# LingmaFuture/PRCV2025REID

Measured on AMD Instinct MI355X. Metric: multimodal instances/sec (PxK, 5-modality) at 1/2/4/8 GPU; eval queries/sec, higher is better.
Workload: dtype bf16; 1 GPU; P=16,K=4 per GPU, vis/nir/sk/cp 224x224 + text (T<=77), CLIP ViT-B/16 + text tower random-init, MER-LoRA r=8, masks all-on, 400 ids, SDM+CE, fwd+bwd+grad sanitise/clip+AdamW (reference default trainable set); P=16, K=4, global_batch=64, lora_rank=8, accum_steps=1, parallelism=dp1

## Files before the change

prcv2025reid_amd/csrc/attention.hip:

```cpp
#include "common.h"
#include <stdlib.h>

namespace {

typedef __attribute__((ext_vector_type(4))) short s4;
typedef __attribute__((address_space(3))) s4* lds_s4_ptr;

constexpr float LOG2E = 1.4426950408889634f;

__device__ __forceinline__ int swz(int row, int c) { return c ^ ((row >> 1) & 7); }

typedef const __attribute__((address_space(1))) void* gptr_t;
typedef __attribute__((address_space(3))) void* lptr_t;

template <int NT>
__device__ __forceinline__ void stage_head(const bf16_t* __restrict__ base, int ld, int S, char* lds, int wave, int lane,
                                           int row_limit = 1 << 30) {
#pragma unroll
    for (int i = 0; i < 4; ++i) {
        const int rblk = (i * NT + wave) * 8;
        if (rblk >= row_limit) continue;
        const int row = rblk + (lane >> 3);
        const int c = swz(row, lane & 7);
        const int grow = row < S ? row : S - 1;
        __builtin_amdgcn_global_load_lds((gptr_t)(base + (size_t)grow * ld + c * 8), (lptr_t)(lds + rblk * 128), 16, 0, 0);
    }
}

__device__ __forceinline__ bf16x8 row_frag(const char* img, int row0, int kchunk, int lane) {
    const int row = row0 + (lane & 31);
    return *(const bf16x8*)(img + row * 128 + (swz(row, kchunk + (lane >> 5)) << 4));
}

__device__ __forceinline__ bf16x8 col_frag(const char* img, int krow0, int col0, int lane) {
    const int h = lane >> 5, half16 = (lane >> 4) & 1, i = lane & 15;
    const int q = i >> 2, pp = i & 3;
    const int col = col0 + 16 * half16 + 4 * pp;
    const int r_lo = krow0 + 4 * h + q, r_hi = r_lo + 8;
    const char* a_lo = img + r_lo * 128 + (swz(r_lo, col >> 3) << 4) + (col & 7) * 2;
    const char* a_hi = img + r_hi * 128 + (swz(r_hi, col >> 3) << 4) + (col & 7) * 2;
    const s4 lo = __builtin_amdgcn_ds_read_tr16_b64_v4i16((lds_s4_ptr)a_lo);
    const s4 hi = __builtin_amdgcn_ds_read_tr16_b64_v4i16((lds_s4_ptr)a_hi);
    return bf16x8{lo[0], lo[1], lo[2], lo[3], hi[0], hi[1], hi[2], hi[3]};
}

__device__ __forceinline__ bf16x8 gfrag(const bf16_t* __restrict__ base, int ld, int row, int kchunk, int lane) {
    return *(const bf16x8*)(base + (size_t)row * ld + (kchunk + (lane >> 5)) * 8);
}

struct FragOff {
    int row[4];
    int col_lo[2];
    int col_hi[2];
};
__device__ __forceinline__ FragOff make_frag_off(int lane) {
    FragOff f;
    const int r = lane & 31, h = lane >> 5;
#pragma unroll
    for (int ks = 0; ks < 4; ++ks) f.row[ks] = r * 128 + (swz(r, 2 * ks + h) << 4);
    const int half16 = (lane >> 4) & 1, i = lane & 15, q = i >> 2, pp = i & 3;
    const int r_lo = 4 * h + q, r_hi = r_lo + 8;
#pragma unroll
    for (int dt = 0; dt < 2; ++dt) {
        const int col = dt * 32 + 16 * half16 + 4 * pp;
        f.col_lo[dt] = r_lo * 128 + (swz(r_lo, col >> 3) << 4) + (col & 7) * 2;
        f.col_hi[dt] = r_hi * 128 + (swz(r_hi, col >> 3) << 4) + (col & 7) * 2;
    }
    return f;
}
__device__ __forceinline__ bf16x8 row_frag_o(const char* img, int tile_row0, int ks, const FragOff& f) {
    return *(const bf16x8*)(img + tile_row0 * 128 + f.row[ks]);
}
__device__ __forceinline__ bf16x8 col_frag_o(const char* img, int krow0, int dt, const FragOff& f) {
    const s4 lo = __builtin_amdgcn_ds_read_tr16_b64_v4i16((lds_s4_ptr)(img + krow0 * 128 + f.col_lo[dt]));
    const s4 hi = __builtin_amdgcn_ds_read_tr16_b64_v4i16((lds_s4_ptr)(img + krow0 * 128 + f.col_hi[dt]));
    return bf16x8{lo[0], lo[1], lo[2], lo[3], hi[0], hi[1], hi[2], hi[3]};
}
__device__ __forceinline__ float fast_exp2(float x) { return __builtin_amdgcn_exp2f(x); }

__device__ __forceinline__ bf16x8 pack8(const f32x16& a, int s) {
    bf16x8 r;
#pragma unroll
    for (int j = 0; j < 8; ++j) r[j] = (short)f32_to_bf16(a[8 * s + j]);
    return r;
}

__device__ __forceinline__ int acc_row(int reg, int lane) { return (reg & 3) + 8 * (reg >> 2) + 4 * (lane >> 5); }

struct AttnParams {
    const bf16_t* qkv; int ld; const uint8_t* key_mask;
    bf16_t* out; int ldo; float* lse;
    const bf16_t* dout; bf16_t* dqkv; int lddqkv; float* delta;
    int n_seq, S, heads, causal;
    int q_tiles;
};

__device__ __forceinline__ void store_tile_row16(bf16_t* row, bool ok, const f32x16& t, float scale, int lane) {
#pragma unroll
    for (int j = 0; j < 2; ++j) {
        const int a = 8 * j, b = 8 * j + 4;
        const auto r0 = __builtin_amdgcn_permlane32_swap(pack_bf16x2(t[a] * scale, t[a + 1] * scale),
                                                         pack_bf16x2(t[b] * scale, t[b + 1] * scale), false, false);
        const auto r1 = __builtin_amdgcn_permlane32_swap(pack_bf16x2(t[a + 2] * scale, t[a + 3] * scale),
                                                         pack_bf16x2(t[b + 2] * scale, t[b + 3] * scale), false, false);
        if (ok) *(uint4*)(row + 8 * (2 * j + (lane >> 5))) = uint4{r0[0], r1[0], r0[1], r1[1]};
    }
}


template <int NT, bool TWO_PASS>
__global__ __launch_bounds__(NT * 64, TWO_PASS ? 4 : 1) void attn_fwd_kernel(const AttnParams p) {
    REID_T16_ENTER();
    extern __shared__ __attribute__((aligned(16))) char smem[];
    char* Ks = smem;
    char* Vs = smem + NT * 32 * 128;
    const int tid = threadIdx.x, lane = tid & 63;
    const int wave = __builtin_amdgcn_readfirstlane(tid >> 6);
    const int seq = blockIdx.x / p.heads, head = blockIdx.x % p.heads;
    const int d = p.heads * 64;
    const bf16_t* qb = p.qkv + (size_t)seq * p.S * p.ld + head * 64;
    stage_head<NT>(qb + d, p.ld, p.S, Ks, wave, lane);
    const int q0 = wave * 32;
    const int qi = q0 + (lane & 31);
    const int qrow = qi < p.S ? qi : p.S - 1;
    bf16x8 qf[4];
#pragma unroll
    for (int ks = 0; ks < 4; ++ks) qf[ks] = gfrag(qb, p.ld, qrow, 2 * ks, lane);
    stage_head<NT>(qb + 2 * d, p.ld, p.S, Vs, wave, lane);
    __syncthreads();
    if (q0 >= p.S || (p.q_tiles > 0 && wave >= p.q_tiles)) return;

    const FragOff fo = make_frag_off(lane);
    const uint8_t* km = p.key_mask ? p.key_mask + (size_t)seq * p.S : nullptr;
    const int h4 = 4 * (lane >> 5);
    const bool general = km != nullptr || p.causal;
    auto score_tile = [&](int kt) -> f32x16 {
        f32x16 t;
#pragma unroll
        for (int e = 0; e < 16; ++e) t[e] = 0.f;
#pragma unroll
        for (int ks = 0; ks < 4; ++ks) t = mfma32(row_frag_o(Ks, kt * 32, ks, fo), qf[ks], t);
        if (general) {
#pragma unroll
            for (int e = 0; e < 16; ++e) {
                const int key = kt * 32 + (e & 3) + 8 * (e >> 2) + h4;
                bool ok = key < p.S;
                if (ok && km) ok = km[key] != 0;
                if (p.causal) ok = ok && key <= qi;
                t[e] = ok ? t[e] : -INFINITY;
            }
        } else if (kt == NT - 1) {
#pragma unroll
            for (int e = 0; e < 16; ++e) {
                const int key = kt * 32 + (e & 3) + 8 * (e >> 2) + h4;
                t[e] = key < p.S ? t[e] : -INFINITY;
            }
        }
        return t;
    };
    const float c = 0.125f * LOG2E;
    f32x16 ot[2];
#pragma unroll
    for (int dt = 0; dt < 2; ++dt)
#pragma unroll
        for (int e = 0; e < 16; ++e) ot[dt][e] = 0.f;
    float mx = -INFINITY, l = 0.f;
    if (TWO_PASS) {
#pragma unroll 1
        for (int kt = 0; kt < NT; ++kt) {
            const f32x16 t = score_tile(kt);
#pragma unroll
            for (int e = 0; e < 16; e += 2) mx = fmaxf(mx, fmaxf(t[e], t[e + 1]));
        }
        mx = fmaxf(mx, __shfl_xor(mx, 32, 64));
        if (mx == -INFINITY) mx = 0.f;
        const float nmc = -mx * c;
#pragma unroll 1
        for (int kt = 0; kt < NT; ++kt) {
            f32x16 t = score_tile(kt);
#pragma unroll
            for (int e = 0; e < 16; ++e) {
                const float pe = fast_exp2(fmaf(t[e], c, nmc));
                t[e] = pe;
                l += pe;
            }
#pragma unroll
            for (int s2 = 0; s2 < 2; ++s2) {
                const bf16x8 pf = pack8(t, s2);
#pragma unroll
                for (int dt = 0; dt < 2; ++dt) ot[dt] = mfma32(col_frag_o(Vs, kt * 32 + 16 * s2, dt, fo), pf, ot[dt]);
            }
        }
    } else {
        f32x16 st[NT];
#pragma unroll
        for (int kt = 0; kt < NT; ++kt) st[kt] = score_tile(kt);
#pragma unroll
        for (int kt = 0; kt < NT; ++kt)
#pragma unroll
            for (int e = 0; e < 16; e += 2) mx = fmaxf(mx, fmaxf(st[kt][e], st[kt][e + 1]));
        mx = fmaxf(mx, __shfl_xor(mx, 32, 64));
        if (mx == -INFINITY) mx = 0.f;
        const float nmc = -mx * c;
#pragma unroll
        for (int kt = 0; kt < NT; ++kt)
#pragma unroll
            for (int e = 0; e < 16; ++e) {
                const float pe = fast_exp2(fmaf(st[kt][e], c, nmc));
                st[kt][e] = pe;
                l += pe;
            }
#pragma unroll
        for (int kt = 0; kt < NT; ++kt)
#pragma unroll
            for (int s2 = 0; s2 < 2; ++s2) {
                const bf16x8 pf = pack8(st[kt], s2);
#pragma unroll
                for (int dt = 0; dt < 2; ++dt) ot[dt] = mfma32(col_frag_o(Vs, kt * 32 + 16 * s2, dt, fo), pf, ot[dt]);
            }
    }
    l += __shfl_xor(l, 32, 64);
    {
        const float inv = 1.0f / l;
        bf16_t* orow = p.out + ((size_t)seq * p.S + qrow) * p.ldo + head * 64;
#pragma unroll
        for (int dt = 0; dt < 2; ++dt) store_tile_row16(orow + dt * 32, qi < p.S, ot[dt], inv, lane);
        if (qi < p.S && p.lse && lane < 32) p.lse[((size_t)seq * p.heads + head) * p.S + qi] = mx * 0.125f + logf(l);
    }
}

template <int NT>
__global__ __launch_bounds__(NT * 64) void attn_bwd_dkv_kernel(const AttnParams p) {
    REID_T16_ENTER();
    extern __shared__ __attribute__((aligned(16))) char smem[];
    char* Qs = smem;
    char* Gs = smem + NT * 32 * 128;
    float* rowc = (float*)(smem + 2 * NT * 32 * 128);
    const int tid = threadIdx.x, lane = tid & 63;
    const int wave = __builtin_amdgcn_readfirstlane(tid >> 6);
    const int seq = blockIdx.x / p.heads, head = blockIdx.x % p.heads;
    const int d = p.heads * 64;
    const bf16_t* qb = p.qkv + (size_t)seq * p.S * p.ld + head * 64;
    const bf16_t* gb = p.dout + (size_t)seq * p.S * p.ldo + head * 64;
    const int q_rows = p.q_tiles > 0 ? p.q_tiles * 32 : NT * 32;
    stage_head<NT>(qb, p.ld, p.S, Qs, wave, lane, q_rows);
    stage_head<NT>(gb, p.ldo, p.S, Gs, wave, lane, q_rows);
    for (int t = tid; t < NT * 32; t += NT * 64) {
        const size_t o = ((size_t)seq * p.heads + head) * p.S + t;
        rowc[t] = t < p.S ? -p.lse[o] * LOG2E : -INFINITY;
        rowc[NT * 32 + t] = t < p.S ? -p.delta[o] * 0.125f : 0.f;
    }
    const int k0 = wave * 32;
    const int ki = k0 + (lane & 31);
    const int krow = ki < p.S ? ki : p.S - 1;
    bf16x8 kf[4], vf[4];
#pragma unroll
    for (int ks = 0; ks < 4; ++ks) {
        kf[ks] = gfrag(qb + d, p.ld, krow, 2 * ks, lane);
        vf[ks] = gfrag(qb + 2 * d, p.ld, krow, 2 * ks, lane);
    }
    __syncthreads();
    if (k0 >= p.S) return;
    const uint8_t* km = p.key_mask ? p.key_mask + (size_t)seq * p.S : nullptr;
    const bool key_ok = ki < p.S && (!km || km[ki] != 0);

    const FragOff fo = make_frag_off(lane);
    f32x16 dkt[2], dvt[2];
#pragma unroll
    for (int dt = 0; dt < 2; ++dt)
#pragma unroll
        for (int e = 0; e < 16; ++e) { dkt[dt][e] = 0.f; dvt[dt][e] = 0.f; }
    const float c = 0.125f * LOG2E;
    const int h4 = 4 * (lane >> 5);
    for (int qt = 0; qt < NT; ++qt) {
        if (qt * 32 >= p.S || (p.q_tiles > 0 && qt >= p.q_tiles)) break;
        f32x16 s, dp;
#pragma unroll
        for (int e = 0; e < 16; ++e) { s[e] = 0.f; dp[e] = 0.f; }
#pragma unroll
        for (int ks = 0; ks < 4; ++ks) {
            s = mfma32(row_frag_o(Qs, qt * 32, ks, fo), kf[ks], s);
            dp = mfma32(row_frag_o(Gs, qt * 32, ks, fo), vf[ks], dp);
        }
        f32x16 pm, ds;
#pragma unroll
        for (int g = 0; g < 4; ++g) {
            const f32x4 nl = *(const f32x4*)(rowc + qt * 32 + 8 * g + h4);
            const f32x4 nd = *(const f32x4*)(rowc + NT * 32 + qt * 32 + 8 * g + h4);
#pragma unroll
            for (int j = 0; j < 4; ++j) {
                const int e = 4 * g + j;
                float pe = fast_exp2(fmaf(s[e], c, nl[j]));
                if (p.causal && ki > qt * 32 + 8 * g + h4 + j) pe = 0.f;
                pm[e] = pe;
                ds[e] = pe * fmaf(dp[e], 0.125f, nd[j]);
            }
        }
#pragma unroll
        for (int s2 = 0; s2 < 2; ++s2) {
            const bf16x8 pf = pack8(pm, s2), df = pack8(ds, s2);
#pragma unroll
            for (int dt = 0; dt < 2; ++dt) {
                dvt[dt] = mfma32(col_frag_o(Gs, qt * 32 + 16 * s2, dt, fo), pf, dvt[dt]);
                dkt[dt] = mfma32(col_frag_o(Qs, qt * 32 + 16 * s2, dt, fo), df, dkt[dt]);
            }
        }
    }
    if (!key_ok) {
#pragma unroll
        for (int dt = 0; dt < 2; ++dt)
#pragma unroll
            for (int e = 0; e < 16; ++e) { dkt[dt][e] = 0.f; dvt[dt][e] = 0.f; }
    }
    {
        const bool ok = ki < p.S;
        bf16_t* drow = p.dqkv + ((size_t)seq * p.S + (ok ? ki : 0)) * p.lddqkv + head * 64;
#pragma unroll
        for (int dt = 0; dt < 2; ++dt) {
            store_tile_row16(drow + d + dt * 32, ok, dkt[dt], 1.0f, lane);
            store_tile_row16(drow + 2 * d + dt * 32, ok, dvt[dt], 1.0f, lane);
        }
    }
}

template <int NT>
__global__ __launch_bounds__(NT * 64) void attn_bwd_dq_kernel(const AttnParams p) {
    REID_T16_ENTER();
    extern __shared__ __attribute__((aligned(16))) char smem[];
    char* Ks = smem;
    char* Vs = smem + NT * 32 * 128;
    const int tid = threadIdx.x, lane = tid & 63;
    const int wave = __builtin_amdgcn_readfirstlane(tid >> 6);
    const int seq = blockIdx.x / p.heads, head = blockIdx.x % p.heads;
    const int d = p.heads * 64;
    const bf16_t* qb = p.qkv + (size_t)seq * p.S * p.ld + head * 64;
    const bf16_t* gb = p.dout + (size_t)seq * p.S * p.ldo + head * 64;
    stage_head<NT>(qb + d, p.ld, p.S, Ks, wave, lane);
    stage_head<NT>(qb + 2 * d, p.ld, p.S, Vs, wave, lane);
    const int q0 = wave * 32;
    const int qi = q0 + (lane & 31);
    const int qrow = qi < p.S ? qi : p.S - 1;
    bf16x8 qf[4], gf[4];
#pragma unroll
    for (int ks = 0; ks < 4; ++ks) {
        qf[ks] = gfrag(qb, p.ld, qrow, 2 * ks, lane);
        gf[ks] = gfrag(gb, p.ldo, qrow, 2 * ks, lane);
    }
    const size_t so = ((size_t)seq * p.heads + head) * p.S + qrow;
    const float nl = -p.lse[so] * LOG2E;
    float dsum = 0.f;
    {
        const bf16_t* ob = p.out + (size_t)seq * p.S * p.ldo + head * 64;
#pragma unroll
        for (int ks = 0; ks < 4; ++ks) {
            const bf16x8 of = gfrag(ob, p.ldo, qrow, 2 * ks, lane);
#pragma unroll
            for (int j = 0; j < 8; ++j) dsum = fmaf(bf16_to_f32((bf16_t)gf[ks][j]), bf16_to_f32((bf16_t)of[j]), dsum);
        }
    }
    dsum += __shfl_xor(dsum, 32, 64);
    if (qi < p.S && lane < 32) p.delta[so] = dsum;
    const float nd = -dsum * 0.125f;
    __syncthreads();
    if (q0 >= p.S) return;
    if (p.q_tiles > 0 && wave >= p.q_tiles) {
        if (qi < p.S) {
            bf16_t* drow = p.dqkv + ((size_t)seq * p.S + qi) * p.lddqkv + head * 64;
#pragma unroll
            for (int dt = 0; dt < 2; ++dt)
#pragma unroll
                for (int g = 0; g < 4; ++g) *(uint2*)(drow + dt * 32 + 8 * g + 4 * (lane >> 5)) = uint2{0u, 0u};
        }
        return;
    }
    const uint8_t* km = p.key_mask ? p.key_mask + (size_t)seq * p.S : nullptr;
    const FragOff fo = make_frag_off(lane);
    f32x16 dqt[2];
#pragma unroll
    for (int dt = 0; dt < 2; ++dt)
#pragma unroll
        for (int e = 0; e < 16; ++e) dqt[dt][e] = 0.f;
    const float c = 0.125f * LOG2E;
    const int h4 = 4 * (lane >> 5);
    const bool slow = km != nullptr || p.causal;
    for (int kt = 0; kt < NT; ++kt) {
        if (kt * 32 >= p.S) break;
        f32x16 s, dp;
#pragma unroll
        for (int e = 0; e < 16; ++e) { s[e] = 0.f; dp[e] = 0.f; }
#pragma unroll
        for (int ks = 0; ks < 4; ++ks) {
            s = mfma32(row_frag_o(Ks, kt * 32, ks, fo), qf[ks], s);
            dp = mfma32(row_frag_o(Vs, kt * 32, ks, fo), gf[ks], dp);
        }
        const bool edge = slow || (kt + 1) * 32 > p.S;
        f32x16 ds;
#pragma unroll
        for (int e = 0; e < 16; ++e) {
            float pe = fast_exp2(fmaf(s[e], c, nl));
            if (edge) {
                const int key = kt * 32 + (e & 3) + 8 * (e >> 2) + h4;
                bool ok = key < p.S;
                if (ok && km) ok = km[key] != 0;
                if (p.causal) ok = ok && key <= qi;
                pe = ok ? pe : 0.f;
            }
            ds[e] = pe * fmaf(dp[e], 0.125f, nd);
        }
#pragma unroll
        for (int s2 = 0; s2 < 2; ++s2) {
            const bf16x8 df = pack8(ds, s2);
#pragma unroll
            for (int dt = 0; dt < 2; ++dt) dqt[dt] = mfma32(col_frag_o(Ks, kt * 32 + 16 * s2, dt, fo), df, dqt[dt]);
        }
    }
    {
        const bool ok = qi < p.S;
        bf16_t* drow = p.dqkv + ((size_t)seq * p.S + (ok ? qi : 0)) * p.lddqkv + head * 64;
#pragma unroll
        for (int dt = 0; dt < 2; ++dt) store_tile_row16(drow + dt * 32, ok, dqt[dt], 1.0f, lane);
    }
}

#ifdef REID_ATTN_TRACE
__device__ unsigned long long* g_attn_bwd_trace = nullptr;
#define ATTN_BWD_STAMP(slot) do { if (g_attn_bwd_trace && threadIdx.x == 0) g_attn_bwd_trace[(size_t)blockIdx.x * 8 + (slot)] = __builtin_amdgcn_s_memrealtime(); } while (0)
#else
#define ATTN_BWD_STAMP(slot) do { } while (0)
#endif
template <int NT>
__global__ __launch_bounds__(NT * 64) void attn_bwd_fused_kernel(const AttnParams p) {
    REID_T16_ENTER();
    ATTN_BWD_STAMP(0);
    extern __shared__ __attribute__((aligned(16))) char smem[];
    constexpr int IMG = NT * 32 * 128;
    char* Qs = smem;
    char* Gs = smem + IMG;
    char* Ks = smem + 2 * IMG;
    char* Vs = smem + 3 * IMG;
    float* rowc = (float*)(smem + 4 * IMG);
    const int tid = threadIdx.x, lane = tid & 63;
    const int wave = __builtin_amdgcn_readfirstlane(tid >> 6);
    const int seq = blockIdx.x / p.heads, head = blockIdx.x % p.heads;
    const int d = p.heads * 64;
    const bf16_t* qb = p.qkv + (size_t)seq * p.S * p.ld + head * 64;
    const bf16_t* gb = p.dout + (size_t)seq * p.S * p.ldo + head * 64;
    const bf16_t* ob = p.out + (size_t)seq * p.S * p.ldo + head * 64;
    const int nq = p.q_tiles > 0 ? (p.q_tiles < NT ? p.q_tiles : NT) : NT;
    const int q_rows = nq * 32;
    stage_head<NT>(qb, p.ld, p.S, Qs, wave, lane, q_rows);
    stage_head<NT>(gb, p.ldo, p.S, Gs, wave, lane, q_rows);
    stage_head<NT>(qb + d, p.ld, p.S, Ks, wave, lane);
    stage_head<NT>(qb + 2 * d, p.ld, p.S, Vs, wave, lane);
    const int t0 = wave * 32;
    const int ti = t0 + (lane & 31);
    const int trow = ti < p.S ? ti : p.S - 1;
    const bool own_q = wave < nq && t0 < p.S;
    bf16x8 of[4];
#pragma unroll
    for (int ks = 0; ks < 4; ++ks) of[ks] = gfrag(ob, p.ldo, trow, 2 * ks, lane);
    const size_t so = ((size_t)seq * p.heads + head) * p.S + trow;
    const float lse_v = p.lse[so];
    const FragOff fo = make_frag_off(lane);
    __syncthreads();
    ATTN_BWD_STAMP(1);
    {
        float dsum = 0.f;
        if (own_q) {
#pragma unroll
            for (int ks = 0; ks < 4; ++ks) {
                const bf16x8 gfk = row_frag_o(Gs, t0, ks, fo);
#pragma unroll
                for (int j = 0; j < 8; ++j) dsum = fmaf(bf16_to_f32((bf16_t)gfk[j]), bf16_to_f32((bf16_t)of[ks][j]), dsum);
            }
        }
        dsum += __shfl_xor(dsum, 32, 64);
        if (lane < 32) {
            const bool live = own_q && ti < p.S;
            rowc[ti] = live ? -lse_v * LOG2E : -INFINITY;
            rowc[NT * 32 + ti] = live ? -dsum * 0.125f : 0.f;
            if (live && p.delta) p.delta[so] = dsum;
        }
    }
    __syncthreads();
    ATTN_BWD_STAMP(2);
    if (t0 >= p.S) return;
    const float c = 0.125f * LOG2E;
    const int h4 = 4 * (lane >> 5);
    const bool tile_ok = ti < p.S;

    {
        bf16x8 kf[4], vf[4];
#pragma unroll
        for (int ks = 0; ks < 4; ++ks) { kf[ks] = row_frag_o(Ks, t0, ks, fo); vf[ks] = row_frag_o(Vs, t0, ks, fo); }
        f32x16 dkt[2], dvt[2];
#pragma unroll
        for (int dt = 0; dt < 2; ++dt)
#pragma unroll
            for (int e = 0; e < 16; ++e) { dkt[dt][e] = 0.f; dvt[dt][e] = 0.f; }
        const int nqt = nq < (p.S + 31) / 32 ? nq : (p.S + 31) / 32;
        auto scores = [&](int qt, f32x16& s, f32x16& dp) {
#pragma unroll
            for (int e = 0; e < 16; ++e) { s[e] = 0.f; dp[e] = 0.f; }
#pragma unroll
            for (int ks = 0; ks < 4; ++ks) {
                s = mfma32(row_frag_o(Qs, qt * 32, ks, fo), kf[ks], s);
                dp = mfma32(row_frag_o(Gs, qt * 32, ks, fo), vf[ks], dp);
            }
        };
        f32x16 s, dp, s_n, dp_n;
        if (nqt > 0) scores(0, s, dp);
        for (int qt = 0; qt < nqt; ++qt) {
            if (qt + 1 < nqt) scores(qt + 1, s_n, dp_n);
#pragma unroll
            for (int s2 = 0; s2 < 2; ++s2) {
                bf16x8 pf, df;
#pragma unroll
                for (int g2 = 0; g2 < 2; ++g2) {
                    const int g = 2 * s2 + g2;
                    const f32x4 nl = *(const f32x4*)(rowc + qt * 32 + 8 * g + h4);
                    const f32x4 nd = *(const f32x4*)(rowc + NT * 32 + qt * 32 + 8 * g + h4);
#pragma unroll
                    for (int j = 0; j < 4; ++j) {
                        const int e = 4 * g + j;
                        const float pe = fast_exp2(fmaf(s[e], c, nl[j]));
                        pf[4 * g2 + j] = (short)f32_to_bf16(pe);
                        df[4 * g2 + j] = (short)f32_to_bf16(pe * fmaf(dp[e], 0.125f, nd[j]));
                    }
                }
#pragma unroll
                for (int dt = 0; dt < 2; ++dt) {
                    dvt[dt] = mfma32(col_frag_o(Gs, qt * 32 + 16 * s2, dt, fo), pf, dvt[dt]);
                    dkt[dt] = mfma32(col_frag_o(Qs, qt * 32 + 16 * s2, dt, fo), df, dkt[dt]);
                }
            }
            s = s_n; dp = dp_n;
        }
        ATTN_BWD_STAMP(3);
        bf16_t* drow = p.dqkv + ((size_t)seq * p.S + trow) * p.lddqkv + head * 64;
#pragma unroll
        for (int dt = 0; dt < 2; ++dt) {
            store_tile_row16(drow + d + dt * 32, tile_ok, dkt[dt], 1.0f, lane);
            store_tile_row16(drow + 2 * d + dt * 32, tile_ok, dvt[dt], 1.0f, lane);
        }
    }

    ATTN_BWD_STAMP(4);
    bf16_t* qrow_out = p.dqkv + ((size_t)seq * p.S + trow) * p.lddqkv + head * 64;
    if (!own_q) {
        if (tile_ok) {
#pragma unroll
            for (int dt = 0; dt < 2; ++dt)
#pragma unroll
                for (int g = 0; g < 4; ++g) *(uint2*)(qrow_out + dt * 32 + 8 * g + 4 * (lane >> 5)) = uint2{0u, 0u};
        }
        return;
    }
    {
        bf16x8 qf[4], gf[4];
#pragma unroll
        for (int ks = 0; ks < 4; ++ks) { qf[ks] = row_frag_o(Qs, t0, ks, fo); gf[ks] = row_frag_o(Gs, t0, ks, fo); }
        const float nl = rowc[ti], nd = rowc[NT * 32 + ti];
        f32x16 dqt[2];
#pragma unroll
        for (int dt = 0; dt < 2; ++dt)
#pragma unroll
            for (int e = 0; e < 16; ++e) dqt[dt][e] = 0.f;
        const int nkt = (p.S + 31) / 32;
        auto scores_t = [&](int kt, f32x16& s, f32x16& dp) {
#pragma unroll
            for (int e = 0; e < 16; ++e) { s[e] = 0.f; dp[e] = 0.f; }
#pragma unroll
            for (int ks = 0; ks < 4; ++ks) {
                s = mfma32(row_frag_o(Ks, kt * 32, ks, fo), qf[ks], s);
                dp = mfma32(row_frag_o(Vs, kt * 32, ks, fo), gf[ks], dp);
            }
        };
        f32x16 s, dp, s_n, dp_n;
        scores_t(0, s, dp);
        for (int kt = 0; kt < nkt; ++kt) {
            if (kt + 1 < nkt) scores_t(kt + 1, s_n, dp_n);
            const bool edge = (kt + 1) * 32 > p.S;
#pragma unroll
            for (int s2 = 0; s2 < 2; ++s2) {
                bf16x8 df;
#pragma unroll
                for (int j = 0; j < 8; ++j) {
                    const int e = 8 * s2 + j;
                    float pe = fast_exp2(fmaf(s[e], c, nl));
                    if (edge) {
                        const int key = kt * 32 + (e & 3) + 8 * (e >> 2) + h4;
                        pe = key < p.S ? pe : 0.f;
                    }
                    df[j] = (short)f32_to_bf16(pe * fmaf(dp[e], 0.125f, nd));
                }
#pragma unroll
                for (int dt = 0; dt < 2; ++dt) dqt[dt] = mfma32(col_frag_o(Ks, kt * 32 + 16 * s2, dt, fo), df, dqt[dt]);
            }
            s = s_n; dp = dp_n;
        }
        ATTN_BWD_STAMP(5);
#pragma unroll
        for (int dt = 0; dt < 2; ++dt) store_tile_row16(qrow_out + dt * 32, tile_ok, dqt[dt], 1.0f, lane);
        ATTN_BWD_STAMP(6);
    }
}

template <int NT>
int launch_fwd(const AttnParams& p, hipStream_t s) {
    constexpr int LDS = 2 * NT * 32 * 128;
    constexpr bool TP = NT >= 4;
    REID_MAX_LDS((attn_fwd_kernel<NT, TP>), LDS);
    hipLaunchKernelGGL((attn_fwd_kernel<NT, TP>), dim3(p.n_seq * p.heads), dim3(NT * 64), LDS, s, p);
    REID_CHECK_LAUNCH("reid_attn_fwd");
    return REID_OK;
}

template <int NT>
int launch_bwd(const AttnParams& p, hipStream_t s) {
    constexpr int LDS1 = 2 * NT * 32 * 128 + 2 * NT * 32 * 4;
    constexpr int LDS2 = 2 * NT * 32 * 128;
    REID_MAX_LDS((attn_bwd_dkv_kernel<NT>), LDS1);
    REID_MAX_LDS((attn_bwd_dq_kernel<NT>), LDS2);
    if (!p.key_mask && !p.causal && reid_knob(KNOB_ATTN_BWD) != 1) {
        constexpr int LDSF = 4 * NT * 32 * 128 + 2 * NT * 32 * 4;
        REID_MAX_LDS((attn_bwd_fused_kernel<NT>), LDSF);
        hipLaunchKernelGGL(attn_bwd_fused_kernel<NT>, dim3(p.n_seq * p.heads), dim3(NT * 64), LDSF, s, p);
        REID_CHECK_LAUNCH("reid_attn_bwd(fused)");
        return REID_OK;
    }
    hipLaunchKernelGGL(attn_bwd_dq_kernel<NT>, dim3(p.n_seq * p.heads), dim3(NT * 64), LDS2, s, p);
    REID_CHECK_LAUNCH("reid_attn_bwd(dq)");
    hipLaunchKernelGGL(attn_bwd_dkv_kernel<NT>, dim3(p.n_seq * p.heads), dim3(NT * 64), LDS1, s, p);
    REID_CHECK_LAUNCH("reid_attn_bwd(dkv)");
    return REID_OK;
}

int check_common(const char* name, const void* qkv, int ld, int n_seq, int S, int heads) {
    REID_CHECK_ARG(qkv != nullptr, "%s: null qkv", name);
    REID_CHECK_ARG(n_seq > 0 && heads > 0 && S > 0 && S <= 224, "%s: S=%d must be in 1..224 (n_seq=%d heads=%d)", name, S, n_seq, heads);
    REID_CHECK_ARG(ld >= 3 * heads * 64 && ld % 8 == 0, "%s: ld=%d must be >= 3*heads*64 and a multiple of 8", name, ld);
    return REID_OK;
}

}

#ifdef REID_ATTN_TRACE
extern "C" void reid_debug_attn_bwd_trace(void* buf) {
    unsigned long long* ptr = (unsigned long long*)buf;
    (void)hipMemcpyToSymbol(HIP_SYMBOL(g_attn_bwd_trace), &ptr, sizeof(ptr));
}
#endif

#define DISPATCH_NT(nt, fn, ...)                \
    switch (nt) {                               \
        case 1: return fn<1>(__VA_ARGS__);      \
        case 2: return fn<2>(__VA_ARGS__);      \
        case 3: return fn<3>(__VA_ARGS__);      \
        case 4: return fn<4>(__VA_ARGS__);      \
        case 5: return fn<5>(__VA_ARGS__);      \
        case 6: return fn<6>(__VA_ARGS__);      \
        default: return fn<7>(__VA_ARGS__);     \
    }

extern "C" int reid_attn_fwd(const void* qkv, int32_t ld, const uint8_t* key_mask, void* out, int32_t ldo, float* lse,
                             int32_t n_seq, int32_t S, int32_t heads, int32_t causal, int32_t q_tiles, void* stream) {
    int rc = check_common("reid_attn_fwd", qkv, ld, n_seq, S, heads);
    if (rc) return rc;
    REID_CHECK_ARG(out && ldo >= heads * 64 && ldo % 4 == 0, "reid_attn_fwd: out/ldo");
    AttnParams p{(const bf16_t*)qkv, ld, key_mask, (bf16_t*)out, ldo, lse, nullptr, nullptr, 0, nullptr, n_seq, S, heads, causal, q_tiles};
    DISPATCH_NT((S + 31) / 32, launch_fwd, p, (hipStream_t)stream)
}

extern "C" int reid_attn_bwd(const void* qkv, int32_t ld, const uint8_t* key_mask, const void* out, const void* dout,
                             int32_t ldo, const float* lse, void* dqkv, int32_t lddqkv, float* delta_ws, int32_t n_seq,
                             int32_t S, int32_t heads, int32_t causal, int32_t q_tiles, void* stream) {
    int rc = check_common("reid_attn_bwd", qkv, ld, n_seq, S, heads);
    if (rc) return rc;
    REID_CHECK_ARG(out && dout && lse && dqkv && delta_ws, "reid_attn_bwd: null pointer");
    REID_CHECK_ARG(ldo >= heads * 64 && ldo % 8 == 0 && lddqkv >= 3 * heads * 64 && lddqkv % 4 == 0, "reid_attn_bwd: ldo/lddqkv");
    AttnParams p{(const bf16_t*)qkv, ld, key_mask, (bf16_t*)out, ldo, (float*)lse, (const bf16_t*)dout, (bf16_t*)dqkv, lddqkv,
                 delta_ws, n_seq, S, heads, causal, q_tiles};
    DISPATCH_NT((S + 31) / 32, launch_bwd, p, (hipStream_t)stream)
}
```

Baseline: 2072 instances/s.

## Reuse dS from dK/dV pass for dQ via LDS transpose reads

The fused attention backward kernel now writes each bf16 dS tile to a swizzled LDS buffer during the dK/dV loop. The dQ pass then reads it back with ds_read_tr16 transposed loads instead of recomputing the S and dP scores and the exponentials. K and V fragments are loaded straight from global memory into registers, and the K tile is staged into LDS only once the Q/G usage ends. This removes half the backward MFMA work and the second exp pass, but costs an S×S LDS buffer, extra barriers, and waves with no tiles no longer exit early.

Measured after the change: 2106 instances/s, median of 6. 1.02x the previous value.

```diff
diff --git a/prcv2025reid_amd/csrc/attention.hip b/prcv2025reid_amd/csrc/attention.hip
--- a/prcv2025reid_amd/csrc/attention.hip
+++ b/prcv2025reid_amd/csrc/attention.hip
@@ -422,6 +422,7 @@
     }
 }
 
+__device__ __forceinline__ int ds_chunk(int r, int c) { return c ^ ((r >> 1) & 3); }
 #ifdef REID_ATTN_TRACE
 __device__ unsigned long long* g_attn_bwd_trace = nullptr;
 #define ATTN_BWD_STAMP(slot) do { if (g_attn_bwd_trace && threadIdx.x == 0) g_attn_bwd_trace[(size_t)blockIdx.x * 8 + (slot)] = __builtin_amdgcn_s_memrealtime(); } while (0)
@@ -434,11 +435,12 @@
     ATTN_BWD_STAMP(0);
     extern __shared__ __attribute__((aligned(16))) char smem[];
     constexpr int IMG = NT * 32 * 128;
+    constexpr int DS_ROW = NT * 64;
     char* Qs = smem;
     char* Gs = smem + IMG;
-    char* Ks = smem + 2 * IMG;
-    char* Vs = smem + 3 * IMG;
-    float* rowc = (float*)(smem + 4 * IMG);
+    char* Ks = smem;
+    char* Ds = smem + 2 * IMG;
+    float* rowc = (float*)(Ds + NT * 32 * DS_ROW);
     const int tid = threadIdx.x, lane = tid & 63;
     const int wave = __builtin_amdgcn_readfirstlane(tid >> 6);
     const int seq = blockIdx.x / p.heads, head = blockIdx.x % p.heads;
@@ -448,14 +450,18 @@
     const bf16_t* ob = p.out + (size_t)seq * p.S * p.ldo + head * 64;
     const int nq = p.q_tiles > 0 ? (p.q_tiles < NT ? p.q_tiles : NT) : NT;
     const int q_rows = nq * 32;
-    stage_head<NT>(qb, p.ld, p.S, Qs, wave, lane, q_rows);
-    stage_head<NT>(gb, p.ldo, p.S, Gs, wave, lane, q_rows);
-    stage_head<NT>(qb + d, p.ld, p.S, Ks, wave, lane);
-    stage_head<NT>(qb + 2 * d, p.ld, p.S, Vs, wave, lane);
     const int t0 = wave * 32;
     const int ti = t0 + (lane & 31);
     const int trow = ti < p.S ? ti : p.S - 1;
-    const bool own_q = wave < nq && t0 < p.S;
+    const bool own_q = wave < nq;
+    bf16x8 kf[4], vf[4];
+#pragma unroll
+    for (int ks = 0; ks < 4; ++ks) {
+        kf[ks] = gfrag(qb + d, p.ld, trow, 2 * ks, lane);
+        vf[ks] = gfrag(qb + 2 * d, p.ld, trow, 2 * ks, lane);
+    }
+    stage_head<NT>(qb, p.ld, p.S, Qs, wave, lane, q_rows);
+    stage_head<NT>(gb, p.ldo, p.S, Gs, wave, lane, q_rows);
     bf16x8 of[4];
 #pragma unroll
     for (int ks = 0; ks < 4; ++ks) of[ks] = gfrag(ob, p.ldo, trow, 2 * ks, lane);
@@ -484,20 +490,20 @@
     }
     __syncthreads();
     ATTN_BWD_STAMP(2);
-    if (t0 >= p.S) return;
     const float c = 0.125f * LOG2E;
     const int h4 = 4 * (lane >> 5);
     const bool tile_ok = ti < p.S;
+    bf16_t* trow_out = p.dqkv + ((size_t)seq * p.S + trow) * p.lddqkv + head * 64;
 
     {
-        bf16x8 kf[4], vf[4];
-#pragma unroll
-        for (int ks = 0; ks < 4; ++ks) { kf[ks] = row_frag_o(Ks, t0, ks, fo); vf[ks] = row_frag_o(Vs, t0, ks, fo); }
         f32x16 dkt[2], dvt[2];
 #pragma unroll
         for (int dt = 0; dt < 2; ++dt)
 #pragma unroll
             for (int e = 0; e < 16; ++e) { dkt[dt][e] = 0.f; dvt[dt][e] = 0.f; }
+        const int hsw = (lane >> 5) ^ (((lane & 31) >> 1) & 3);
+        char* const ds_w0 = Ds + ti * DS_ROW + 16 * hsw;
+        char* const ds_w1 = Ds + ti * DS_ROW + 16 * (hsw ^ 2);
         const int nqt = nq < (p.S + 31) / 32 ? nq : (p.S + 31) / 32;
         auto scores = [&](int qt, f32x16& s, f32x16& dp) {
 #pragma unroll
@@ -533,75 +539,56 @@
                     dvt[dt] = mfma32(col_frag_o(Gs, qt * 32 + 16 * s2, dt, fo), pf, dvt[dt]);
                     dkt[dt] = mfma32(col_frag_o(Qs, qt * 32 + 16 * s2, dt, fo), df, dkt[dt]);
                 }
+                *(bf16x8*)((s2 ? ds_w1 : ds_w0) + qt * 64) = tile_ok ? df : bf16x8{};
             }
             s = s_n; dp = dp_n;
         }
         ATTN_BWD_STAMP(3);
-        bf16_t* drow = p.dqkv + ((size_t)seq * p.S + trow) * p.lddqkv + head * 64;
 #pragma unroll
         for (int dt = 0; dt < 2; ++dt) {
-            store_tile_row16(drow + d + dt * 32, tile_ok, dkt[dt], 1.0f, lane);
-            store_tile_row16(drow + 2 * d + dt * 32, tile_ok, dvt[dt], 1.0f, lane);
-        }
-    }
-
+            store_tile_row16(trow_out + d + dt * 32, tile_ok, dkt[dt], 1.0f, lane);
+            store_tile_row16(trow_out + 2 * d + dt * 32, tile_ok, dvt[dt], 1.0f, lane);
+        }
+    }
+
+    __syncthreads();
+#pragma unroll
+    for (int ks = 0; ks < 4; ++ks) *(bf16x8*)(Ks + t0 * 128 + fo.row[ks]) = kf[ks];
+    __syncthreads();
     ATTN_BWD_STAMP(4);
-    bf16_t* qrow_out = p.dqkv + ((size_t)seq * p.S + trow) * p.lddqkv + head * 64;
+
     if (!own_q) {
         if (tile_ok) {
 #pragma unroll
             for (int dt = 0; dt < 2; ++dt)
 #pragma unroll
-                for (int g = 0; g < 4; ++g) *(uint2*)(qrow_out + dt * 32 + 8 * g + 4 * (lane >> 5)) = uint2{0u, 0u};
+                for (int g = 0; g < 4; ++g) *(uint2*)(trow_out + dt * 32 + 8 * g + 4 * (lane >> 5)) = uint2{0u, 0u};
         }
         return;
     }
     {
-        bf16x8 qf[4], gf[4];
-#pragma unroll
-        for (int ks = 0; ks < 4; ++ks) { qf[ks] = row_frag_o(Qs, t0, ks, fo); gf[ks] = row_frag_o(Gs, t0, ks, fo); }
-        const float nl = rowc[ti], nd = rowc[NT * 32 + ti];
+        const int h = lane >> 5, half16 = (lane >> 4) & 1, q = (lane & 15) >> 2, pp = lane & 3;
+        const int r = 4 * h + q;
+        const int ds_r = r * DS_ROW + 16 * ds_chunk(r, 4 * wave + 2 * half16 + (pp & 1)) + 8 * (pp >> 1);
         f32x16 dqt[2];
 #pragma unroll
         for (int dt = 0; dt < 2; ++dt)
 #pragma unroll
             for (int e = 0; e < 16; ++e) dqt[dt][e] = 0.f;
-        const int nkt = (p.S + 31) / 32;
-        auto scores_t = [&](int kt, f32x16& s, f32x16& dp) {
-#pragma unroll
-            for (int e = 0; e < 16; ++e) { s[e] = 0.f; dp[e] = 0.f; }
-#pragma unroll
-            for (int ks = 0; ks < 4; ++ks) {
-                s = mfma32(row_frag_o(Ks, kt * 32, ks, fo), qf[ks], s);
-                dp = mfma32(row_frag_o(Vs, kt * 32, ks, fo), gf[ks], dp);
-            }
-        };
-        f32x16 s, dp, s_n, dp_n;
-        scores_t(0, s, dp);
-        for (int kt = 0; kt < nkt; ++kt) {
-            if (kt + 1 < nkt) scores_t(kt + 1, s_n, dp_n);
-            const bool edge = (kt + 1) * 32 > p.S;
+#pragma unroll
+        for (int kt = 0; kt < NT; ++kt)
 #pragma unroll
             for (int s2 = 0; s2 < 2; ++s2) {
-                bf16x8 df;
-#pragma unroll
-                for (int j = 0; j < 8; ++j) {
-                    const int e = 8 * s2 + j;
-                    float pe = fast_exp2(fmaf(s[e], c, nl));
-                    if (edge) {
-                        const int key = kt * 32 + (e & 3) + 8 * (e >> 2) + h4;
-                        pe = key < p.S ? pe : 0.f;
-                    }
-                    df[j] = (short)f32_to_bf16(pe * fmaf(dp[e], 0.125f, nd));
-                }
-#pragma unroll
-                for (int dt = 0; dt < 2; ++dt) dqt[dt] = mfma32(col_frag_o(Ks, kt * 32 + 16 * s2, dt, fo), df, dqt[dt]);
-            }
-            s = s_n; dp = dp_n;
-        }
+                const int krow0 = kt * 32 + 16 * s2;
+                const s4 lo = __builtin_amdgcn_ds_read_tr16_b64_v4i16((lds_s4_ptr)(Ds + krow0 * DS_ROW + ds_r));
+                const s4 hi = __builtin_amdgcn_ds_read_tr16_b64_v4i16((lds_s4_ptr)(Ds + (krow0 + 8) * DS_ROW + ds_r));
+                const bf16x8 df = bf16x8{lo[0], lo[1], lo[2], lo[3], hi[0], hi[1], hi[2], hi[3]};
+#pragma unroll
+                for (int dt = 0; dt < 2; ++dt) dqt[dt] = mfma32(col_frag_o(Ks, krow0, dt, fo), df, dqt[dt]);
+            }
         ATTN_BWD_STAMP(5);
 #pragma unroll
-        for (int dt = 0; dt < 2; ++dt) store_tile_row16(qrow_out + dt * 32, tile_ok, dqt[dt], 1.0f, lane);
+        for (int dt = 0; dt < 2; ++dt) store_tile_row16(trow_out + dt * 32, tile_ok, dqt[dt], 1.0f, lane);
         ATTN_BWD_STAMP(6);
     }
 }
@@ -623,7 +610,7 @@
     REID_MAX_LDS((attn_bwd_dkv_kernel<NT>), LDS1);
     REID_MAX_LDS((attn_bwd_dq_kernel<NT>), LDS2);
     if (!p.key_mask && !p.causal && reid_knob(KNOB_ATTN_BWD) != 1) {
-        constexpr int LDSF = 4 * NT * 32 * 128 + 2 * NT * 32 * 4;
+        constexpr int LDSF = 2 * NT * 32 * 128 + (NT * 32) * (NT * 64) + 2 * NT * 32 * 4;
         REID_MAX_LDS((attn_bwd_fused_kernel<NT>), LDSF);
         hipLaunchKernelGGL(attn_bwd_fused_kernel<NT>, dim3(p.n_seq * p.heads), dim3(NT * 64), LDSF, s, p);
         REID_CHECK_LAUNCH("reid_attn_bwd(fused)");
```
